# omricarmi/FastHEVC

Hardware: AMD Instinct MI355X
Metric: CTU depth decisions/sec at 1080p all-intra + BD-rate delta vs full-RDO HM (higher is better)
Workload: dtype int8 operands / int32 accumulate on v_mfma_i32_32x32x32_i8 (conv2, conv3: 93 % of the MACs); conv1 bf16 operands / f32 accumulate (fixed-point valued); every result exact

## Files before the change

### fasthevc_amd/csrc/fhevc_api.hip

```cpp
#include "../../include/fasthevc.h"
#include "fhevc_internal.h"

#include <algorithm>
#include <cmath>
#include <cstdio>
#include <cstdlib>
#include <cstring>
#include <functional>
#include <new>
#include <string>
#include <thread>
#include <vector>

namespace {

struct TimedLaunch { hipEvent_t start, stop; int which; };

}

struct fhevc_ctx {
  fhevc_cfg cfg{};
  int device = 0, num_cus = 256;
  hipStream_t stream = nullptr;
  int ctus_x = 0, ctus_y = 0, num_ctus = 0;
  int dev_stride = 0;
  bool have_weights = false;
  uint4* d_frag = nullptr; float* d_bias = nullptr; uint8_t* d_whead = nullptr; int32_t* d_bhead = nullptr;
  uint4* d_frag_i8 = nullptr; int32_t* d_bias_i8 = nullptr;
  bool family = false;
  bool fam_layers = false;
  bool fam_d2 = false;
  FhevcLayersWeights lw = {};
  std::vector<void*> lw_bufs;
  hipEvent_t lw_done = nullptr; hipStream_t lw_last_stream = nullptr; bool lw_in_flight = false;
  int fam_c[3] = { 0, 0, 0 };
  uint4* f_frag1 = nullptr; float* f_bias1 = nullptr; uint4* f_frag2 = nullptr; uint4* f_frag3 = nullptr; int32_t* f_bias_i8 = nullptr;
  uint8_t* f_whead = nullptr; uint8_t* f_headm = nullptr; int32_t* f_bhead = nullptr;
  int shift[3] = { 0, 0, 0 };
  int requant_mode[3] = { 0, 0, 0 };
  bool cnn_i8 = true;
  float scale[3] = { 1, 1, 1 };
  int16_t* d_luma = nullptr; uint8_t* d_depth = nullptr; int32_t* d_had = nullptr; FhevcNodeCost* d_nodes = nullptr;
  int16_t* d_satd = nullptr; uint32_t* d_satd_out = nullptr;
  hipEvent_t ev[4] = { nullptr, nullptr, nullptr, nullptr };
  bool fuse_hadamard = true;
  bool motion_sad = false;
  bool had_valu = true;
  FhevcKnobs knobs;
  bool timing = false;
  std::vector<TimedLaunch> pending;
  std::vector<std::pair<hipEvent_t, hipEvent_t>> pool;
  double sum_ms[5] = { 0, 0, 0, 0, 0 };
  uint64_t launches[5] = { 0, 0, 0, 0, 0 };
  double* d_act = nullptr;
  int16_t* d_pair = nullptr;
  FhevcMotionNode* d_motion = nullptr;
  FhevcNodeCost* d_cand_all = nullptr; uint8_t* d_cand = nullptr;
  uint32_t* d_mvtab = nullptr;
  int mvtab_qp = -1, mvtab_range = -1;
  hipEvent_t mvtab_used = nullptr;
  std::vector<uint32_t> mvtab_host;
  struct Slot {
    hipStream_t st = nullptr;
    uint8_t* d_in = nullptr; uint8_t* d_depth = nullptr; int32_t* d_had = nullptr;
    uint8_t* h_in = nullptr; uint8_t* h_depth = nullptr; int32_t* h_had = nullptr;
    size_t in_cap = 0, frames_cap = 0, h_in_cap = 0;
    int frames = 0; uint8_t* out_depth = nullptr; int32_t* out_had = nullptr; bool staged_out = false;
  } slot[2];
  uint8_t* d_depth_max = nullptr;
  fhevc_stats stats{};
  std::string err;
  std::vector<fhevc_ctx*> peers;
  int fail_peer_for_test = -1;
};

namespace {

int fail(fhevc_ctx* c, int code, const char* what, hipError_t e = hipSuccess)
{
  if (c) {
    c->err = what;
// ... 105 lines not shown
          const int col = 4 * h + (j >> 1), row = 2 * st - 1 + (j & 1);
          uint16_t bits = 0;
          if (c != 0 && row >= 0 && row <= 7) bits = ((__builtin_popcount(u & row) + __builtin_popcount(v & col)) & 1) ? 0xBF80 : 0x3F80;
          frag[((size_t)FHEVC_FRAG_HAD + (mt * 5 + st) * 64 + lane) * 8 + j] = bits;
        }
      }
  std::vector<int8_t> frag8((size_t)FHEVC_FRAGI8_TOTAL * 16, 0);
  for (int lane = 0; lane < 64; ++lane) {
    const int r = lane & 31, h = lane >> 5;
    for (int j = 0; j < 16; ++j) {
      auto w2 = [&](int ky, int kx) { return b.w2[(r * 16 + j) * 9 + ky * 3 + kx]; };
      int8_t* f2 = &frag8[((size_t)FHEVC_FRAGI8_CONV2 + lane) * 16 + j];
      for (int kx = 0; kx < 3; ++kx) f2[(size_t)kx * 1024] = w2(h, kx);
      f2[3 * 1024] = w2(2, 2 * h);
      f2[4 * 1024] = h == 0 ? w2(2, 1) : 0;
      f2[5 * 1024] = h == 1 ? w2(2, 1) : 0;
      for (int t = 0; t < 2; ++t)
        for (int tap = 0; tap < 9; ++tap)
          frag8[((size_t)FHEVC_FRAGI8_CONV3 + (t * 9 + tap) * 64 + lane) * 16 + j] = b.w3[((32 * t + r) * 32 + 16 * h + j) * 9 + tap];
    }
  }
  std::vector<int32_t> bias8(112, 0);
  long long bound[3] = { 0, 0, 0 };
  for (int oc = 0; oc < 32; ++oc) {
    int sw = 0, sa = 0;
    for (int i = 0; i < 16 * 9; ++i) { sw += b.w2[oc * 144 + i]; sa += std::abs((int)b.w2[oc * 144 + i]); }
    bias8[16 + oc] = rd32(b.b2, oc) + 128 * sw;
    bound[1] = std::max(bound[1], (long long)std::abs(bias8[16 + oc]) + 128LL * sa);
  }
  for (int oc = 0; oc < 64; ++oc) {
    int sw = 0, sa = 0;
    for (int i = 0; i < 32 * 9; ++i) { sw += b.w3[oc * 288 + i]; sa += std::abs((int)b.w3[oc * 288 + i]); }
    bias8[48 + oc] = rd32(b.b3, oc) + 128 * sw;
    bound[2] = std::max(bound[2], (long long)std::abs(bias8[48 + oc]) + 128LL * sa);
  }
  for (int l = 1; l < 3; ++l) {
    const int sh = rd32(b.shift, l);
    new_mode[l] = c->knobs.requant_general ? 0 : (sh == 8 && bound[l] < (1LL << 23)) ? 2 : (sh <= 7 ? 1 : 0);
  }
  std::vector<float> bias(112);
  for (int i = 0; i < 16; ++i) {
    int sw = 0;
    for (int t = 0; t < 9; ++t) sw += b.w1[i * 9 + t];
    if (std::abs(rd32(b.b1, i)) > 4194304) return fail(c, FHEVC_E_WEIGHTS, "|bias| > 2^22");
    bias[i] = (float)(rd32(b.b1, i) - 128 * sw);
  }
  for (int i = 0; i < 32; ++i) bias[16 + i] = (float)rd32(b.b2, i);
  for (int i = 0; i < 64; ++i) bias[48 + i] = (float)rd32(b.b3, i);
  for (int i = 16; i < 112; ++i) if (std::fabs(bias[i]) > 4194304.0f) return fail(c, FHEVC_E_WEIGHTS, "|bias| > 2^22");
  std::vector<uint8_t> whead(4 * 4096 + 2 * 1024);
  for (int i = 0; i < 8192; ++i) whead[i] = (uint8_t)b.wh64[i];
  for (int i = 0; i < 8192; ++i) whead[8192 + i] = (uint8_t)b.wh32[i];
  for (int i = 0; i < 2048; ++i) whead[16384 + i] = (uint8_t)b.wh16[i];
  int32_t bhead[6 + 3 * 52] = { rd32(b.bh64, 0), rd32(b.bh64, 1), rd32(b.bh32, 0), rd32(b.bh32, 1), rd32(b.bh16, 0), rd32(b.bh16, 1) };
  for (int cls = 0; cls < 2; ++cls) {
    int s64 = 0, s32 = 0, s16 = 0;
    for (int i = 0; i < 4096; ++i) { s64 += b.wh64[cls * 4096 + i]; s32 += b.wh32[cls * 4096 + i]; }
    for (int i = 0; i < 1024; ++i) s16 += b.wh16[cls * 1024 + i];
    bhead[0 + cls] += 128 * 4 * s64;
    bhead[2 + cls] += 128 * s32;
    bhead[4 + cls] += 128 * s16;
  }
  for (int i = 0; i < 3 * 52; ++i) bhead[6 + i] = rd32(b.qp_bias, i);

  if (c->have_weights && !c->family) c->have_weights = false;
  if (!c->d_frag) {
    HIP_TRY(c, hipMalloc(&c->d_frag, frag.size() * 2));
    HIP_TRY(c, hipMalloc(&c->d_bias, bias.size() * 4));
    HIP_TRY(c, hipMalloc(&c->d_whead, whead.size()));
    HIP_TRY(c, hipMalloc(&c->d_bhead, sizeof bhead));
    HIP_TRY(c, hipMalloc(&c->d_frag_i8, frag8.size()));
    HIP_TRY(c, hipMalloc(&c->d_bias_i8, bias8.size() * 4));
  }
  HIP_TRY(c, hipMemcpy(c->d_frag_i8, frag8.data(), frag8.size(), hipMemcpyHostToDevice));
  HIP_TRY(c, hipMemcpy(c->d_bias_i8, bias8.data(), bias8.size() * 4, hipMemcpyHostToDevice));
  HIP_TRY(c, hipMemcpy(c->d_frag, frag.data(), frag.size() * 2, hipMemcpyHostToDevice));
  HIP_TRY(c, hipMemcpy(c->d_bias, bias.data(), bias.size() * 4, hipMemcpyHostToDevice));
  HIP_TRY(c, hipMemcpy(c->d_whead, whead.data(), whead.size(), hipMemcpyHostToDevice));
  HIP_TRY(c, hipMemcpy(c->d_bhead, bhead, sizeof bhead, hipMemcpyHostToDevice));
  for (int l = 0; l < 3; ++l) { c->shift[l] = new_shift[l]; c->scale[l] = std::ldexp(1.0f, -new_shift[l]); c->requant_mode[l] = new_mode[l]; }
  c->family = false; c->fam_layers = false;
  c->have_weights = true;
  return FHEVC_OK;
}

int build_layers_image(fhevc_ctx* c, const uint8_t* blob, size_t bytes, int C1, int C2, int C3, int depth)
{
  const int C[3] = { C1, C2, C3 };
  for (int b = 0; b < 3; ++b) if (C[b] < 1 || C[b] > 128) return fail(c, FHEVC_E_WEIGHTS, "family widths must be 1..128");
  if (depth < 1 || depth > 3 || (C3 & 3)) return fail(c, FHEVC_E_WEIGHTS, "family members: 1..3 convolutions per block, last width a multiple of 4");
  size_t need = 24 + 36, ci = 1;
  for (int b = 0; b < 3; ++b) for (int j = 0; j < depth; ++j) { need += (size_t)C[b] * ci * 9 + 4 * (size_t)C[b]; ci = (size_t)C[b]; }
  need += (size_t)(2 * 64 + 2 * 64 + 2 * 16) * C3 + 24 + 3 * 52 * 4;
  if (bytes != need) return fail(c, FHEVC_E_WEIGHTS, "FHW3 blob has the wrong size");
  size_t off = 24;
  auto take = [&](size_t n) { const uint8_t* q = blob + off; off += n; return q; };
  auto i32at = [](const uint8_t* p, int i) { int32_t v; std::memcpy(&v, p + 4 * (size_t)i, 4); return v; };
  int32_t shift33[9];
  std::memcpy(shift33, take(36), 36);
  {
    size_t o = off, cin_v = 1;
    for (int b = 0; b < 3; ++b)
      for (int j = 0; j < depth; ++j) {
        const size_t nw = (size_t)C[b] * cin_v * 9;
        for (size_t i = 0; i < nw; ++i) if (static_cast<int8_t>(blob[o + i]) == -128) return fail(c, FHEVC_E_WEIGHTS, "weight -128 not allowed");
        o += nw + 4 * (size_t)C[b];
        cin_v = (size_t)C[b];
        if (shift33[b * 3 + j] < 0 || shift33[b * 3 + j] > 14) return fail(c, FHEVC_E_WEIGHTS, "shift out of range (0..14)");
      }
    const size_t head_bytes[3] = { (size_t)2 * 64 * C3, (size_t)2 * 64 * C3, (size_t)2 * 16 * C3 };
    for (int hd = 0; hd < 3; ++hd) {
      for (size_t i = 0; i < head_bytes[hd]; ++i) if (blob[o + i] == 0x80) return fail(c, FHEVC_E_WEIGHTS, "weight -128 not allowed");
      o += head_bytes[hd] + 8;
    }
  }
  for (void* q : c->lw_bufs) (void)hipFree(q);
  c->lw_bufs.clear();
  if (c->family && c->fam_layers) c->have_weights = false;
  FhevcLayersWeights lw = {};
  lw.chunk = std::min(c->num_ctus * std::max(1, c->cfg.max_frames), 8192);
  if (lw.chunk < 64) lw.chunk = 64;
  auto dev = [&](size_t n, int fill) -> void* { void* q = nullptr; if (hipMalloc(&q, n) != hipSuccess) return nullptr; c->lw_bufs.push_back(q); (void)hipMemset(q, fill, n); return q; };
  auto pad32 = [](int v) { return 32 * ((v + 31) / 32); };
  const bool d2 = depth == 2 && pad32(C1) == 32 && pad32(C2) == 64 && pad32(C3) == 96 && c->knobs.fused_d2 && !c->knobs.family_layers;
  if (!d2 && !(lw.in0 = static_cast<int8_t*>(dev((size_t)lw.chunk * 66 * 66, 0)))) return fail(c, FHEVC_E_HIP, "layer buffers");
  int H = 64, cin = 1, li = 0;
// ... 179 lines not shown
        const int8_t* src;
        if (n < 2) src = wh16 + ((size_t)n * 16 + j) * C3 + 64 * kc;
        else {
          const int sub = (n - 2) >> 1, cls = n & 1, py = j >> 2, px = j & 3;
          src = wh32 + ((size_t)cls * 64 + ((sub >> 1) * 4 + py) * 8 + (sub & 1) * 4 + px) * C3 + 64 * kc;
        }
        std::memcpy(headm.data() + (((size_t)j * KC + kc) * 16 + n) * 64, src, 64);
      }
  int32_t bhead[6 + 3 * 52] = { i32at(bh64p, 0), i32at(bh64p, 1), i32at(bh32p, 0), i32at(bh32p, 1), i32at(bh16p, 0), i32at(bh16p, 1) };
  for (int cls = 0; cls < 2; ++cls) {
    int s64 = 0, s32 = 0, s16 = 0;
    for (int i = 0; i < 64 * C3; ++i) { s64 += wh64[(size_t)cls * 64 * C3 + i]; s32 += wh32[(size_t)cls * 64 * C3 + i]; }
    for (int i = 0; i < 16 * C3; ++i) s16 += wh16[(size_t)cls * 16 * C3 + i];
    bhead[0 + cls] += 128 * 4 * s64;
    bhead[2 + cls] += 128 * s32;
    bhead[4 + cls] += 128 * s16;
  }
  for (int i = 0; i < 3 * 52; ++i) bhead[6 + i] = i32at(qpb, i);
  if (c->family && !c->fam_layers) c->have_weights = false;
  (void)hipFree(c->f_frag1); (void)hipFree(c->f_bias1); (void)hipFree(c->f_frag2); (void)hipFree(c->f_frag3); (void)hipFree(c->f_bias_i8); (void)hipFree(c->f_whead); (void)hipFree(c->f_headm); (void)hipFree(c->f_bhead);
  c->f_frag1 = nullptr; c->f_headm = nullptr; c->f_bias1 = nullptr; c->f_frag2 = nullptr; c->f_frag3 = nullptr; c->f_bias_i8 = nullptr; c->f_whead = nullptr; c->f_bhead = nullptr;
  HIP_TRY(c, hipMalloc(&c->f_frag1, frag1.size() * 2)); HIP_TRY(c, hipMalloc(&c->f_bias1, bias1.size() * 4));
  HIP_TRY(c, hipMalloc(&c->f_frag2, frag2.size())); HIP_TRY(c, hipMalloc(&c->f_frag3, frag3.size()));
  HIP_TRY(c, hipMalloc(&c->f_bias_i8, bias8.size() * 4)); HIP_TRY(c, hipMalloc(&c->f_whead, whead.size())); HIP_TRY(c, hipMalloc(&c->f_headm, headm.size())); HIP_TRY(c, hipMalloc(&c->f_bhead, sizeof bhead));
  HIP_TRY(c, hipMemcpy(c->f_frag1, frag1.data(), frag1.size() * 2, hipMemcpyHostToDevice));
  HIP_TRY(c, hipMemcpy(c->f_bias1, bias1.data(), bias1.size() * 4, hipMemcpyHostToDevice));
  HIP_TRY(c, hipMemcpy(c->f_frag2, frag2.data(), frag2.size(), hipMemcpyHostToDevice));
  HIP_TRY(c, hipMemcpy(c->f_frag3, frag3.data(), frag3.size(), hipMemcpyHostToDevice));
  HIP_TRY(c, hipMemcpy(c->f_bias_i8, bias8.data(), bias8.size() * 4, hipMemcpyHostToDevice));
  HIP_TRY(c, hipMemcpy(c->f_whead, whead.data(), whead.size(), hipMemcpyHostToDevice));
  HIP_TRY(c, hipMemcpy(c->f_headm, headm.data(), headm.size(), hipMemcpyHostToDevice));
  HIP_TRY(c, hipMemcpy(c->f_bhead, bhead, sizeof bhead, hipMemcpyHostToDevice));
  c->fam_c[0] = C1; c->fam_c[1] = C2; c->fam_c[2] = C3;
  c->shift[0] = sh[0]; c->shift[1] = sh[1]; c->shift[2] = sh[2];
  c->family = true; c->fam_layers = false;
  c->have_weights = true;
  return FHEVC_OK;
}

FhevcFamilyWeights family_weights(const fhevc_ctx* c)
{
  FhevcFamilyWeights w;
  w.c[0] = c->fam_c[0]; w.c[1] = c->fam_c[1]; w.c[2] = c->fam_c[2];
  w.frag1 = c->f_frag1; w.bias1 = c->f_bias1; w.frag2 = c->f_frag2; w.frag3 = c->f_frag3; w.bias_i8 = c->f_bias_i8; w.whead = c->f_whead; w.headm = c->f_headm; w.bhead = c->f_bhead;
  w.shift[0] = c->shift[0]; w.shift[1] = c->shift[1]; w.shift[2] = c->shift[2];
  return w;
}

FhevcCnnWeights cnn_weights(const fhevc_ctx* c)
{
  FhevcCnnWeights w;
  w.frag = c->d_frag; w.bias = c->d_bias; w.whead = c->d_whead; w.bhead = c->d_bhead;
  w.scale[0] = c->scale[0]; w.scale[1] = c->scale[1]; w.scale[2] = c->scale[2];
  w.frag_i8 = c->d_frag_i8; w.bias_i8 = c->d_bias_i8;
  w.shift[0] = c->shift[0]; w.shift[1] = c->shift[1]; w.shift[2] = c->shift[2];
  w.requant_mode[0] = 0; w.requant_mode[1] = c->requant_mode[1]; w.requant_mode[2] = c->requant_mode[2];
  w.i8 = c->cnn_i8 ? 1 : 0;
  w.had_valu = c->had_valu ? 1 : 0;
  return w;
}

void time_begin(fhevc_ctx* c, hipStream_t s, int which)
{
  if (!c->timing) return;
  TimedLaunch t;
  if (!c->pool.empty()) { t.start = c->pool.back().first; t.stop = c->pool.back().second; c->pool.pop_back(); }
  else { (void)hipEventCreate(&t.start); (void)hipEventCreate(&t.stop); }
  t.which = which;
  (void)hipEventRecord(t.start, s);
  c->pending.push_back(t);
}
void time_end(fhevc_ctx* c, hipStream_t s)
{
  if (!c->timing) return;
  (void)hipEventRecord(c->pending.back().stop, s);
}
void time_resolve(fhevc_ctx* c)
{
  for (auto& t : c->pending) {
    float ms = 0;
    if (hipEventSynchronize(t.stop) == hipSuccess && hipEventElapsedTime(&ms, t.start, t.stop) == hipSuccess) {
      c->sum_ms[t.which] += ms;
      c->launches[t.which] += 1;
      if (t.which == 0) c->stats.last_cnn_ms = ms;
      if (t.which == 1) c->stats.last_hadamard_ms = ms;
      if (t.which == 2) c->stats.last_first_pass_ms = ms;
    }
    c->pool.emplace_back(t.start, t.stop);
  }
  c->pending.clear();
}

FhevcFrames frames_of(const fhevc_ctx* c, const void* d_luma, int sample_bytes, int stride, long long frame_stride,
                      int num_frames, int row_begin, int row_end, int qp = 32)
{
  FhevcFrames f;
  f.luma = d_luma; f.sample_bytes = sample_bytes; f.stride = stride; f.frame_stride = frame_stride;
  f.width = c->cfg.width; f.height = c->cfg.height; f.bit_depth = c->cfg.bit_depth;
  f.ctus_x = c->ctus_x; f.ctus_y = c->ctus_y; f.num_frames = num_frames; f.row_begin = row_begin; f.row_end = row_end;
  f.qp = qp < 0 ? 0 : (qp > 51 ? 51 : qp);
  return f;
}

}

extern "C" {

// ... 39 lines not shown
  c->ctus_y = (cfg->height + 63) / 64;
  c->num_ctus = c->ctus_x * c->ctus_y;
  c->dev_stride = c->ctus_x * 64;
  if (hipStreamCreateWithFlags(&c->stream, hipStreamDefault) != hipSuccess) { delete c; return FHEVC_E_NO_DEVICE; }
  if (fhevc_cnn_prepare_device() != hipSuccess) { (void)hipStreamDestroy(c->stream); delete c; return FHEVC_E_NO_DEVICE; }
  bool ok = true;
  ok &= hipMalloc(&c->d_luma, (size_t)c->dev_stride * c->ctus_y * 64 * sizeof(int16_t)) == hipSuccess;
  ok &= hipMalloc(&c->d_depth, (size_t)c->num_ctus * 256) == hipSuccess;
  ok &= hipMalloc(&c->d_had, (size_t)c->num_ctus * 4) == hipSuccess;
  ok &= hipMalloc(&c->d_nodes, (size_t)c->num_ctus * FHEVC_NODES_PER_CTU * sizeof(FhevcNodeCost)) == hipSuccess;
  ok &= hipMalloc(&c->d_satd, 2 * 64 * 64 * sizeof(int16_t)) == hipSuccess;
  ok &= hipMalloc(&c->d_satd_out, 4) == hipSuccess;
  for (auto& e : c->ev) ok &= hipEventCreate(&e) == hipSuccess;
  if (!ok) { fhevc_destroy(c); return FHEVC_E_NOMEM; }
  if (hipMemset(c->d_luma, 0, (size_t)c->dev_stride * c->ctus_y * 64 * sizeof(int16_t)) != hipSuccess) { fhevc_destroy(c); return FHEVC_E_HIP; }
  if (cfg->weights_path) {
    FILE* fp = std::fopen(cfg->weights_path, "rb");
    if (!fp) { fhevc_destroy(c); return FHEVC_E_WEIGHTS; }
    std::vector<uint8_t> buf((size_t)4 << 20);
    const size_t n = std::fread(buf.data(), 1, buf.size(), fp);
    std::fclose(fp);
    const int rc = fhevc_set_weights(c, buf.data(), n);
    if (rc != FHEVC_OK) { fhevc_destroy(c); return rc; }
  }
  c->stats.devices = 1;
  for (int d = 1; d < cfg->num_devices; ++d) {
    fhevc_cfg sub = *cfg;
    int id = cfg->device_ids[d];
    sub.num_devices = 1;
    sub.device_ids = &id;
    fhevc_ctx* peer = nullptr;
    if (fhevc_create(&peer, &sub) == FHEVC_OK) { c->peers.push_back(peer); c->stats.devices++; }
    else c->stats.devices_failed++;
  }
  if (const char* ft = std::getenv("FHEVC_TEST_FAIL_DEVICE")) c->fail_peer_for_test = std::atoi(ft);
  (void)hipSetDevice(c->device);
  *out = c;
  return FHEVC_OK;
}

void fhevc_destroy(fhevc_ctx* c)
{
  if (!c) return;
  for (fhevc_ctx* peer : c->peers) fhevc_destroy(peer);
  c->peers.clear();
  (void)hipSetDevice(c->device);
  if (c->stream) (void)hipStreamSynchronize(c->stream);
  time_resolve(c);
  for (auto& p : c->pool) { (void)hipEventDestroy(p.first); (void)hipEventDestroy(p.second); }
  for (auto& e : c->ev) if (e) (void)hipEventDestroy(e);
  if (c->lw_done) (void)hipEventDestroy(c->lw_done);
  if (c->mvtab_used) (void)hipEventDestroy(c->mvtab_used);
  (void)hipFree(c->d_frag); (void)hipFree(c->d_bias); (void)hipFree(c->d_whead); (void)hipFree(c->d_bhead);
  (void)hipFree(c->d_frag_i8); (void)hipFree(c->d_bias_i8);
  (void)hipFree(c->f_frag1); (void)hipFree(c->f_bias1); (void)hipFree(c->f_frag2); (void)hipFree(c->f_frag3); (void)hipFree(c->f_bias_i8); (void)hipFree(c->f_whead); (void)hipFree(c->f_headm); (void)hipFree(c->f_bhead);
  (void)hipFree(c->d_luma); (void)hipFree(c->d_depth); (void)hipFree(c->d_had); (void)hipFree(c->d_nodes); (void)hipFree(c->d_satd); (void)hipFree(c->d_satd_out); (void)hipFree(c->d_act); (void)hipFree(c->d_depth_max); (void)hipFree(c->d_pair); (void)hipFree(c->d_motion); (void)hipFree(c->d_mvtab); (void)hipFree(c->d_cand_all); (void)hipFree(c->d_cand);
  for (void* q : c->lw_bufs) (void)hipFree(q);
  for (auto& sl : c->slot) {
    if (sl.st) { (void)hipStreamSynchronize(sl.st); (void)hipStreamDestroy(sl.st); }
    (void)hipFree(sl.d_in); (void)hipFree(sl.d_depth); (void)hipFree(sl.d_had);
    if (sl.h_in) (void)hipHostFree(sl.h_in);
    if (sl.h_depth) (void)hipHostFree(sl.h_depth);
    if (sl.h_had) (void)hipHostFree(sl.h_had);
  }
  if (c->stream) (void)hipStreamDestroy(c->stream);
  delete c;
}

int fhevc_set_weights(fhevc_ctx* c, const void* blob, size_t bytes)
{
  if (!c || !blob) return FHEVC_E_INVALID;
  auto push_to_peers = [&]() {
    for (fhevc_ctx* peer : c->peers) {
      const int rc = fhevc_set_weights(peer, blob, bytes);
      if (rc != FHEVC_OK) {
        c->have_weights = false;
        for (fhevc_ctx* p2 : c->peers) p2->have_weights = false;
        return fail(c, rc, "weights rejected by a peer device");
      }
    }
    (void)hipSetDevice(c->device);
    return (int)FHEVC_OK;
  };
  (void)hipSetDevice(c->device);
  if (bytes >= 4 && std::memcmp(blob, "FHW3", 4) == 0) {
    const int rc = build_family_image(c, static_cast<const uint8_t*>(blob), bytes);
    return rc != FHEVC_OK ? rc : push_to_peers();
  }
  BlobView v;
  std::vector<uint8_t> copy;
  if (!parse_blob(static_cast<const uint8_t*>(blob), bytes, v, copy)) return fail(c, FHEVC_E_WEIGHTS, "not an FHW1 blob");
  const struct { const int8_t* p; size_t n; } i8s[6] = { { v.w1, 144 }, { v.w2, 4608 }, { v.w3, 18432 }, { v.wh64, 8192 }, { v.wh32, 8192 }, { v.wh16, 2048 } };
  for (const auto& a : i8s)
    for (size_t i = 0; i < a.n; ++i) if (a.p[i] == -128) return fail(c, FHEVC_E_WEIGHTS, "weight -128 not allowed");
  const int rc = build_weight_image(c, v);
  return rc != FHEVC_OK ? rc : push_to_peers();
}

int fhevc_enable_kernel_timing(fhevc_ctx* c, int on)
{
  if (!c) return FHEVC_E_INVALID;
  if (!on) time_resolve(c);
  c->timing = on != 0;
  return FHEVC_OK;
}

int fhevc_kernel_timing(fhevc_ctx* c, int which, int reset, double* avg_ms, uint64_t* launches)
// ... 884 lines not shown
```

### fasthevc_amd/csrc/fhevc_internal.h

```cpp
#pragma once
#include <hip/hip_runtime.h>
#include <stdint.h>

#define FHEVC_CTU 64

#define FHEVC_FRAG_CONV1 0
#define FHEVC_FRAG_CONV2 128
#define FHEVC_FRAG_CONV3 (128 + 9 * 64)
#define FHEVC_FRAG_HAD (128 + 9 * 64 + 2 * 18 * 64)
#define FHEVC_FRAG_TOTAL (FHEVC_FRAG_HAD + 2 * 5 * 64)
#ifndef FHEVC_F16_CONV3_32
#define FHEVC_F16_CONV3_32 0
#endif
#define FHEVC_STAMP_SLOTS 11
#define FHEVC_FRAGI8_CONV2 0
#define FHEVC_FRAGI8_CONV3 (6 * 64)
#define FHEVC_FRAGI8_TOTAL (6 * 64 + 2 * 9 * 64)

struct FhevcKnobs {
  int wg_per_cu = 0;
  int debug_wg_per_cu = 0;
  bool requant_general = false;
  bool family_layers = false;
  bool trio = false;
  bool d2_requant_general = false;
  bool fused_d2 = true;
  bool layers_no_fuse = false;
  bool layers_no_dbuf = false;
  size_t layers_lds_limit = 80 * 1024;
  int layers_grid = 2048;
};
FhevcKnobs fhevc_read_knobs();

struct FhevcFrames {
  const void* luma;
  int sample_bytes;
  int stride;
  long long frame_stride;
  int width, height, bit_depth;
  int ctus_x, ctus_y;
  int num_frames;
  int row_begin, row_end;
  int qp;
};

struct FhevcCnnWeights {
  const uint4* frag;
  const float* bias;
  const uint8_t* whead;
  const int32_t* bhead;
  float scale[3];
  const uint4* frag_i8;
  const int32_t* bias_i8;
  int shift[3];
  int requant_mode[3];
  int i8;
  int had_valu;
};

struct FhevcFamilyWeights {
  int c[3];
  const uint4* frag1;
  const float* bias1;
  const uint4* frag2;
  const uint4* frag3;
  const int32_t* bias_i8;
  const uint8_t* whead;
  const uint8_t* headm;
  const int32_t* bhead;
  int shift[3];
};
hipError_t fhevc_launch_cnn_family(const FhevcFrames& fr, const FhevcFamilyWeights& w, uint8_t* d_depth, int32_t* d_logits, uint32_t* d_flags,
                                   uint8_t* d_depth_max, int margin_split, int margin_stop, int num_cus, hipStream_t stream);
bool fhevc_cnn_family_supported(int c1, int c2, int c3);

struct FhevcLayer {
  const uint4* frag;
  const int32_t* bias;
  int8_t* out;
  int shift, kc, cout_pad, H, pool;
  int rq;
  int in_pad, out_pad, swz;
};
void fhevc_layer_lds_image(int kc, int pool, int H, int* pad, int* mask);
struct FhevcLayersWeights {
  int num_layers, chunk, c3, c3_pad;
  int d2_short;
  FhevcLayer l[9];
  int8_t* in0;
  const uint8_t* whead;
  const int32_t* bhead;
};

hipError_t fhevc_launch_cnn_layers(const FhevcFrames& fr, const FhevcLayersWeights& w, uint8_t* d_depth, int32_t* d_logits, uint32_t* d_flags,
                                   uint8_t* d_depth_max, int margin_split, int margin_stop, int num_cus, const FhevcKnobs& knobs, hipStream_t stream);

bool fhevc_cnn_d2_supported(const FhevcLayersWeights& w);
hipError_t fhevc_launch_cnn_d2(const FhevcFrames& fr, const FhevcLayersWeights& w, uint8_t* d_depth, int32_t* d_logits, uint32_t* d_flags,
                               uint8_t* d_depth_max, int margin_split, int margin_stop, int num_cus, hipStream_t stream);

hipError_t fhevc_cnn_prepare_device();
bool fhevc_cnn_can_fuse_hadamard(const FhevcFrames& fr);
hipError_t fhevc_launch_cnn(const FhevcFrames& fr, const FhevcCnnWeights& w, uint8_t* d_depth, int32_t* d_had, int32_t* d_logits,
                            uint32_t* d_flags, uint8_t* d_depth_max, int margin_split, int margin_stop, int num_cus, const FhevcKnobs& knobs, hipStream_t stream);
hipError_t fhevc_launch_expand_flags(const FhevcFrames& fr, const uint32_t* d_flags, uint8_t* d_depth, hipStream_t stream);

// ... 36 lines not shown
```

### fasthevc_amd/csrc/k_cnn.hip

```cpp
#include "fhevc_internal.h"
#include <algorithm>
#include <cstdlib>
#include <cstring>

typedef __attribute__((ext_vector_type(8))) short bf16x8;
typedef __attribute__((ext_vector_type(8))) _Float16 f16x8;
typedef __attribute__((ext_vector_type(16))) float f32x16;
typedef __attribute__((ext_vector_type(2))) unsigned short u16x2;

namespace {

constexpr int A1_ROW = 36 * 16;
constexpr int A1_EVEN = 19 * 16;
constexpr int R1_OFF = 0;
constexpr int A3_OFF = R1_OFF;
constexpr int A2_PITCH = 18;
constexpr int A2_PLANE = 18 * 18 * 16 + 192;
constexpr int IN_PITCH = 68;
#ifndef FHEVC_I8_PRIO
#define FHEVC_I8_PRIO 0x0222
#endif
#ifndef FHEVC_F16_PRIO
#define FHEVC_F16_PRIO 0x0123
#endif
// ... 552 lines not shown
  const u16x2 sh = { (unsigned short)shift, (unsigned short)shift };
  t = __builtin_bit_cast(s16x2, (u16x2)((__builtin_bit_cast(u16x2, t) + __builtin_bit_cast(u16x2, rnd2)) >> sh));
  t = __builtin_elementwise_min(t, top);
  return __builtin_bit_cast(unsigned, t);
}

template <bool HALO = true>
__device__ __forceinline__ void stage_ctu(unsigned char* lds, int r2_off, const Prefetched& pre, const FhevcFrames& F, CtuPos c,
                                          int tid, int ld_row, int ld_seg, int shift_in, unsigned in_cells)
{
  unsigned short* inh = reinterpret_cast<unsigned short*>(lds + r2_off);
  const int hy = ld_row + 1;
  unsigned short* dst = inh + 2 * ((hy >> 1) * IN_PITCH + ld_seg * 16 + 1) + (hy & 1);
  if (pre.fast) {
    if (F.sample_bytes == 2) {
      const unsigned wds[8] = { pre.a.x, pre.a.y, pre.a.z, pre.a.w, pre.b.x, pre.b.y, pre.b.z, pre.b.w };
      const unsigned rnd2 = shift_in > 0 ? (0x00010001u << (shift_in - 1)) : 0u;
#pragma unroll
      for (int j = 0; j < 8; ++j) {
        const unsigned t = sample8_pair(wds[j], shift_in, rnd2);
        dst[4 * j] = (unsigned short)(__float_as_uint((float)(t & 0xFF)) >> 16);
        dst[4 * j + 2] = (unsigned short)(__float_as_uint((float)((t >> 16) & 0xFF)) >> 16);
      }
    } else {
      const unsigned wds[4] = { pre.a.x, pre.a.y, pre.a.z, pre.a.w };
#pragma unroll
      for (int j = 0; j < 16; ++j) {
        const unsigned v = (wds[j >> 2] >> (8 * (j & 3))) & 0xFF;
        dst[2 * j] = (unsigned short)(__float_as_uint((float)v) >> 16);
      }
    }
  } else {
    const int f = c.f, cy = F.row_begin + c.ry, cx = c.cx;
    const int py = cy * 64 + ld_row, px0 = cx * 64 + ld_seg * 16;
    const long long base = (long long)f * F.frame_stride + (long long)py * F.stride + px0;
    const bool row_ok = py < F.height;
#pragma unroll 4
    for (int j = 0; j < 16; ++j) {
      int v = 128;
      if (row_ok && px0 + j < F.width) {
        if (F.sample_bytes == 2) v = load_sample8(reinterpret_cast<const int16_t*>(F.luma) + base + j, shift_in);
        else v = (int)reinterpret_cast<const uint8_t*>(F.luma)[base + j];
      }
      dst[2 * j] = (unsigned short)(__float_as_uint((float)v) >> 16);
    }
  }
  if (HALO) {
    asm volatile("" : "+v"(in_cells));
    *reinterpret_cast<unsigned short*>(lds + (in_cells & 0xFFFF)) = 0x4300;
    if (tid < 260 - 256) *reinterpret_cast<unsigned short*>(lds + (in_cells >> 16)) = 0x4300;
  }
}
template <bool I8>
__device__ __forceinline__ int a1_halo_off(int e)
{
  const int pl = e / 132, k0 = e - pl * 132;
  int y, x;
  if (k0 < 34) { y = 0; x = k0; }
  else if (k0 < 68) { y = 33; x = k0 - 34; }
  else { const int k = k0 - 68; y = 1 + (k >> 1); x = (k & 1) ? 33 : 0; }
  return R1_OFF + pl * Lds<I8>::A1_PLANE + y * A1_ROW + ((x & 1) ? 0 : A1_EVEN) + (x >> 1) * 16;
}
template <bool I8>
__device__ __forceinline__ int a2_halo_off(int e)
{
  const int pl = e / 68, k0 = e - pl * 68;
  int y, x;
  if (k0 < 18) { y = 0; x = k0; }
  else if (k0 < 36) { y = 17; x = k0 - 18; }
  else { const int k = k0 - 36; y = 1 + (k >> 1); x = (k & 1) ? 17 : 0; }
  return Lds<I8>::R2_OFF + pl * A2_PLANE + (y * A2_PITCH + x) * 16;
}
template <bool I8>
__device__ __forceinline__ int in_halo_off(int e)
{
  int y, x;
  if (e < 66) { y = 0; x = e; }
  else if (e < 132) { y = 65; x = e - 66; }
  else { const int k = e - 132; y = 1 + (k >> 1); x = (k & 1) ? 65 : 0; }
  return Lds<I8>::R2_OFF + 2 * (2 * ((y >> 1) * IN_PITCH + x) + (y & 1));
}
struct HaloCells { unsigned a1, a2, in; };
template <bool I8>
__device__ __forceinline__ HaloCells halo_cells(int tid)
{
  constexpr int N1 = 132 * Lds<I8>::A1_PLANES, N2 = 68 * Lds<I8>::A2_PLANES;
  HaloCells hc;
  hc.a1 = (unsigned)a1_halo_off<I8>(min(tid, N1 - 1)) | ((unsigned)a1_halo_off<I8>(min(tid + 256, N1 - 1)) << 16);
  hc.a2 = (unsigned)a2_halo_off<I8>(min(tid, N2 - 1)) | ((unsigned)a2_halo_off<I8>(min(tid + 256, N2 - 1)) << 16);
  hc.in = (unsigned)in_halo_off<I8>(tid) | ((unsigned)in_halo_off<I8>(min(tid + 256, 259)) << 16);
  return hc;
}
template <bool I8>
__device__ __forceinline__ void zero_a1_halo(unsigned char* lds, int tid, unsigned cells)
{
  asm volatile("" : "+v"(cells));
  constexpr unsigned Z = Lds<I8>::HALO_FILL;
  *reinterpret_cast<uint4*>(lds + (cells & 0xFFFF)) = make_uint4(Z, Z, Z, Z);
  if (tid < 132 * Lds<I8>::A1_PLANES - 256) *reinterpret_cast<uint4*>(lds + (cells >> 16)) = make_uint4(Z, Z, Z, Z);
}

__device__ __forceinline__ unsigned long long stamp()
{
  unsigned long long t;
  __builtin_amdgcn_sched_barrier(0);
  asm volatile("s_memtime %0\n\ts_waitcnt lgkmcnt(0)" : "=s"(t)::"memory");
  __builtin_amdgcn_sched_barrier(0);
  return t;
}

#define FHEVC_PHASE_IDS                                   \
  int tid = (int)threadIdx.x;                             \
  asm volatile("" : "+v"(tid));                           \
  if (TRIO) tid &= 255;                                   \
  const int lane = tid & 63, wave = tid >> 6;             \
  const int r = lane & 31, h = lane >> 5;                 \
  (void)r; (void)h; (void)wave;

template <bool STAMPS, int HAD, int ARITH, int TRIO = 0>
__global__ __launch_bounds__(TRIO ? 768 : 256, TRIO ? 1 : (ARITH ? FHEVC_I8_WG_PER_CU : 2)) void fhevc_cnn_depth_kernel(FhevcFrames F, FhevcCnnWeights W,
                                                                  uint8_t* __restrict__ d_depth, int32_t* __restrict__ d_had,
                                                                  int32_t* __restrict__ d_logits,
                                                                  uint32_t* __restrict__ d_flags,
                                                                  unsigned long long* __restrict__ d_stamps,
                                                                  uint8_t* __restrict__ d_depth_max, int margin_split, int margin_stop)
{
  extern __shared__ __attribute__((aligned(16))) unsigned char lds_all[];
  const int group = TRIO ? __builtin_amdgcn_readfirstlane((int)(threadIdx.x >> 8)) : 0;
  unsigned char* const lds = lds_all + (TRIO ? group * Lds<ARITH != 0>::LDS_BYTES : 0);
  const int vgrid = TRIO ? 3 * (int)gridDim.x : (int)gridDim.x;
  const int vbidx = TRIO ? group * (int)gridDim.x + (int)blockIdx.x : (int)blockIdx.x;
  __builtin_amdgcn_s_setreg((1 << 11) | 1, 2);
  const int tid = TRIO ? (int)(threadIdx.x & 255) : (int)threadIdx.x;
  const int lane = tid & 63, wave = tid >> 6;
  constexpr bool I8 = ARITH != 0, FASTRQ = ARITH == 2;
  int prio_slot = 0;
  if (I8) {
    const unsigned la = __builtin_amdgcn_s_getreg((31 << 11) | 6);
    const unsigned base = la & 0xFFFu, sz = (la >> 12) & 0x1FFu;
    prio_slot = base >= 2 * sz && sz ? 2 : (base >= sz && sz ? 1 : 0);
    if (TRIO) prio_slot = group;
  }
  (void)prio_slot;
  constexpr bool MFMA_HEADS = I8;
  (void)FASTRQ;
  using L = Lds<I8>;
  const HaloCells hc = halo_cells<I8>(tid);
  const int hb64a = W.bhead[0], hb64b = W.bhead[1] + W.bhead[6 + 0 * 52 + F.qp];
  const int hb32a = W.bhead[2], hb32b = W.bhead[3] + W.bhead[6 + 1 * 52 + F.qp];
  const int hb16a = W.bhead[4], hb16b = W.bhead[5] + W.bhead[6 + 2 * 52 + F.qp];
  const uint4* frag1p = W.frag + FHEVC_FRAG_CONV1 + lane;
  bf16x8 wA1a = __builtin_bit_cast(bf16x8, frag1p[0]);
  bf16x8 wA1b = __builtin_bit_cast(bf16x8, frag1p[64]);
  bf16x8 wA2[9];
  bf16x8 wA3[18];
  const int tile3 = wave & 1;
  if (I8) {
#pragma unroll
    for (int s = 0; s < 6; ++s) wA2[s] = __builtin_bit_cast(bf16x8, W.frag_i8[FHEVC_FRAGI8_CONV2 + s * 64 + lane]);
#pragma unroll
    for (int s = 0; s < 9; ++s) wA3[s] = __builtin_bit_cast(bf16x8, W.frag_i8[FHEVC_FRAGI8_CONV3 + (tile3 * 9 + s) * 64 + lane]);
  } else {
#pragma unroll
    for (int s = 0; s < 9; ++s) wA2[s] = __builtin_bit_cast(bf16x8, W.frag[FHEVC_FRAG_CONV2 + s * 64 + lane]);
#pragma unroll
    for (int s = 0; s < 18; ++s) wA3[s] = __builtin_bit_cast(bf16x8, W.frag[FHEVC_FRAG_CONV3 + (tile3 * 18 + s) * 64 + lane]);
  }
  const int shift2 = W.shift[1], shift3 = W.shift[2];
  (void)shift2; (void)shift3;

  float* biasL = reinterpret_cast<float*>(lds + L::BIAS_OFF);
  int* logitL = reinterpret_cast<int*>(lds + L::LOGIT_OFF);
  if (tid < 112) {
    if (I8 && tid >= 16) {
      reinterpret_cast<int*>(biasL)[tid] = W.bias_i8[tid];
    } else {
      float b = W.bias[tid];
      b *= (tid < 16 ? W.scale[0] : (tid < 48 ? W.scale[1] : W.scale[2]));
      biasL[tid] = b;
    }
  }
  for (int i = tid; i < (MFMA_HEADS ? 8192 : 18432) / 16; i += 256) {
    const int row = i >> 2, c = i & 3;
    const int sw = (i < 2 * 4096 * 2 / 16) ? ((row >> 3) & 3) : ((row >> 2) & 3);
    *reinterpret_cast<uint4*>(lds + L::HEADW_OFF + row * 64 + ((c ^ sw) << 4)) = reinterpret_cast<const uint4*>(W.whead)[i];
  }
  if (MFMA_HEADS) {
    for (int i = tid; i < HEADM_BYTES / 16; i += 256) {
      const int j = i / 40, rem = i - j * 40, n = rem >> 2, kg = rem & 3;
      int src;
      if (n < 2) src = 16384 + (n * 16 + j) * 64;
      else {
        const int sub = (n - 2) >> 1, cls = n & 1, py = j >> 2, px = j & 3;
        src = 8192 + (cls * 64 + ((sub >> 1) * 4 + py) * 8 + (sub & 1) * 4 + px) * 64;
      }
      *reinterpret_cast<uint4*>(lds + L::HEADW_OFF + HEADM_OFF + i * 16) = *reinterpret_cast<const uint4*>(W.whead + src + kg * 16);
    }
  }

  if (MFMA_HEADS && tid < 64) {
    const int n = tid & 15, rg = tid >> 4, subn = (n - 2) >> 1;
    const bool is16 = n < 2, is32 = n >= 2 && n < 10 && ((rg & 1) == (subn >> 1));
    unsigned a[4];
    for (int i = 0; i < 4; ++i) {
      const bool act = is16 || (is32 && ((i & 1) == (subn & 1)));
      const int idx = is16 ? 2 * (5 + 4 * rg + i) + n : 2 * (1 + (rg >> 1) * 2 + (i >> 1)) + (n & 1);
      a[i] = act ? (unsigned)(L::LOGIT_OFF + 4 * idx) : (unsigned)(L::HEADX_OFF + 512 + 4 * tid);
    }
    *reinterpret_cast<uint2*>(lds + L::HEADX_OFF + tid * 8) = make_uint2(a[0] | (a[1] << 16), a[2] | (a[3] << 16));
  }
  const int band_rows = F.row_end - F.row_begin;
  const int per_frame = band_rows * F.ctus_x;
  const int total = per_frame * F.num_frames;
  const int shift_in = F.bit_depth - 8;

  unsigned long long tsum[8] = { 0, 0, 0, 0, 0, 0, 0, 0 }, tprev = 0;
#define FHEVC_STAMP(k)                                     \
  if (STAMPS) {                                            \
    const unsigned long long tn = stamp();                 \
    tsum[k] += tn - tprev;                                 \
    tprev = tn;                                            \
  }
  unsigned long long tclk0 = 0, treal0 = 0;
  if (STAMPS) {
    tprev = stamp();
    tclk0 = tprev;
    asm volatile("s_memrealtime %0\n\ts_waitcnt lgkmcnt(0)" : "=s"(treal0)::"memory");
  }

  const int ld_row = tid >> 2, ld_seg = tid & 3;
  const int vblock = (vgrid & 7) ? vbidx : ((vbidx & 7) * (vgrid >> 3) + (vbidx >> 3));
  CtuPos pos, step;
  {
    const int vb = min(vblock, total - 1), g = vgrid;
    pos.f = vb / per_frame; pos.ry = (vb - pos.f * per_frame) / F.ctus_x; pos.cx = (vb - pos.f * per_frame) - pos.ry * F.ctus_x;
    step.f = g / per_frame; step.ry = (g - step.f * per_frame) / F.ctus_x; step.cx = (g - step.f * per_frame) - step.ry * F.ctus_x;
  }
  Prefetched pre = prefetch_ctu<HAD == 1>(F, vblock < total, pos, ld_row, ld_seg);
  uint2 head_addr;
  {
    const int q = wave, blk = lane >> 4;
    const int y = (q >> 1) * 8 + (blk >> 1) * 4 + ((lane >> 2) & 3), x = (q & 1) * 8 + (blk & 1) * 4 + (lane & 3);
    const unsigned psw = (x >> 2) & 3, sw16 = y & 3, sw32 = y & 3, sw64 = (y >> 1) & 3;
    const unsigned a_0 = (unsigned)(y * 16 + x) * 64 + (psw << 4);
    const unsigned w16_0 = (unsigned)((y & 3) * 4 + (x & 3)) * 64 + (sw16 << 4);
    const unsigned w32_0 = (unsigned)((y & 7) * 8 + (x & 7)) * 64 + (sw32 << 4);
    const unsigned w64_0 = (unsigned)((y >> 1) * 8 + (x >> 1)) * 64 + (sw64 << 4);
    head_addr = make_uint2(a_0 | (w16_0 << 16), w32_0 | (w64_0 << 16));
  }
  unsigned headm_addr = 0;
  if (MFMA_HEADS) {
    const int m = lane & 15, kg = lane >> 4, by = m >> 2, bx = m & 3;
    const unsigned am = (unsigned)((4 * by + wave) * 16 + 4 * bx) * 64 + ((unsigned)(kg ^ bx) << 4);
    const unsigned bm = (unsigned)(HEADM_OFF + 4 * wave * HEADM_STEP + min(m, 9) * 64 + 16 * kg);
    headm_addr = am | (bm << 16);
  }
  (void)headm_addr;
  int had_set = 0;
  if (vblock < total) {
    stage_ctu(lds, L::R2_OFF, pre, F, pos, tid, ld_row, ld_seg, shift_in, hc.in);
    zero_a1_halo<I8>(lds, tid, hc.a1);
    if (HAD == 1) {
      const int hs = F.sample_bytes == 2 ? wave_src_hadamard<2>(pre, lane) : wave_src_hadamard<1>(pre, lane);
      if (lane == 0) logitL[56 + wave] = hs;
    }
  }
  __syncthreads();
  FHEVC_STAMP(0)
  float4 early_b0, early_b1;
  bf16x8 early_bq;
#define FHEVC_CONV1_EARLY_READS                                                                          \
  {                                                                                                      \
    FHEVC_PHASE_IDS                                                                                      \
    early_b0 = *reinterpret_cast<const float4*>(biasL + 8 * h);                                          \
    early_b1 = *reinterpret_cast<const float4*>(biasL + 8 * h + 4);                                      \
    const unsigned char* p = lds + L::R2_OFF + (2 * r + 2 * h) * 4 + wave * (IN_PITCH * 4);              \
    const uint2 lo = *reinterpret_cast<const uint2*>(p);                                                 \
    const uint2 hi = *reinterpret_cast<const uint2*>(p + IN_PITCH * 4);                                  \
    early_bq = __builtin_bit_cast(bf16x8, make_uint4(lo.x, lo.y, hi.x, hi.y));                           \
  }
  FHEVC_CONV1_EARLY_READS
  bf16x8 wH[5];
#define FHEVC_HAD_FRAG_LOADS                                                                                                              \
  if (HAD == 2) {                                                                                                                         \
    unsigned hoff = (unsigned)(threadIdx.x & 63) * 16u + (unsigned)((threadIdx.x >> 6) & 1) * (5u * 64u * 16u);   \
    asm volatile("" : "+v"(hoff));                                                                                                        \
    const unsigned char* hf = reinterpret_cast<const unsigned char*>(W.frag + FHEVC_FRAG_HAD) + hoff;                                     \
    _Pragma("unroll") for (int st = 0; st < 5; ++st) wH[st] = __builtin_bit_cast(bf16x8, *reinterpret_cast<const uint4*>(hf + st * 64 * 16)); \
  }
  FHEVC_HAD_FRAG_LOADS

  if (TRIO) {
    for (int i = 0; i < group; ++i) __syncthreads();
  }
  const int trio_iters = TRIO ? (total + vgrid - 1) / vgrid : 0;
  for (int work = vblock, it = 0; TRIO ? it < trio_iters : work < total; work += vgrid, ++it) {
    if (TRIO && work >= total) {
      __syncthreads(); __syncthreads(); __syncthreads(); __syncthreads();
      continue;
    }
    const int f = pos.f, cy = F.row_begin + pos.ry, cx = pos.cx;
    const CtuPos next = advance(pos, step, band_rows, F.ctus_x);


    {
      FHEVC_PHASE_IDS
      FHEVC_PRIO_ON(0)
      const unsigned char* inb = lds + L::R2_OFF + (2 * r + 2 * h) * 4;
      f32x16 bias1;
      {
        const float4 b0 = early_b0, b1 = early_b1;
        bias1[0] = b0.x; bias1[1] = b0.y; bias1[2] = b0.z; bias1[3] = b0.w;
        bias1[4] = b1.x; bias1[5] = b1.y; bias1[6] = b1.z; bias1[7] = b1.w;
#pragma unroll
        for (int i = 0; i < 8; ++i) bias1[8 + i] = bias1[i];
      }
      auto frag1 = [](const unsigned char* p) {
        const uint2 lo = *reinterpret_cast<const uint2*>(p);
        const uint2 hi = *reinterpret_cast<const uint2*>(p + IN_PITCH * 4);
// ... 714 lines not shown
```

Baseline: 85.81 million.

## Pre-swizzle head weights on host and DMA them into LDS with global_load_lds

The MFMA-heads path now receives a head-weight image whose swizzle is computed once on the host. It is copied into LDS with direct global-to-LDS loads, replacing the per-thread load/swizzle/store loops. Halo offsets and head-index tables become constexpr device tables instead of being computed per thread. The CTU prefetch is moved earlier so it overlaps with weight staging. The cost is an extra device buffer and a full vmcnt wait before the first barrier, which may serialize the prefetch.

```diff
diff --git a/fasthevc_amd/csrc/fhevc_api.hip b/fasthevc_amd/csrc/fhevc_api.hip
--- a/fasthevc_amd/csrc/fhevc_api.hip
+++ b/fasthevc_amd/csrc/fhevc_api.hip
@@ -27,6 +27,7 @@
   bool have_weights = false;
   uint4* d_frag = nullptr; float* d_bias = nullptr; uint8_t* d_whead = nullptr; int32_t* d_bhead = nullptr;
   uint4* d_frag_i8 = nullptr; int32_t* d_bias_i8 = nullptr;
+  uint4* d_headimg = nullptr;
   bool family = false;
   bool fam_layers = false;
   bool fam_d2 = false;
@@ -238,6 +239,21 @@
   for (int i = 0; i < 8192; ++i) whead[i] = (uint8_t)b.wh64[i];
   for (int i = 0; i < 8192; ++i) whead[8192 + i] = (uint8_t)b.wh32[i];
   for (int i = 0; i < 2048; ++i) whead[16384 + i] = (uint8_t)b.wh16[i];
+  std::vector<uint8_t> headimg(FHEVC_HEADIMG_BYTES);
+  for (int i = 0; i < 8192 / 16; ++i) {
+    const int row = i >> 2, ch = i & 3, sw = (row >> 3) & 3;
+    std::memcpy(headimg.data() + row * 64 + ((ch ^ sw) << 4), whead.data() + 16 * i, 16);
+  }
+  for (int j = 0; j < 16; ++j)
+    for (int n = 0; n < 10; ++n) {
+      int src;
+      if (n < 2) src = 16384 + (n * 16 + j) * 64;
+      else {
+        const int sub = (n - 2) >> 1, cls = n & 1, py = j >> 2, px = j & 3;
+        src = 8192 + (cls * 64 + ((sub >> 1) * 4 + py) * 8 + (sub & 1) * 4 + px) * 64;
+      }
+      std::memcpy(headimg.data() + 8192 + (j * 10 + n) * 64, whead.data() + src, 64);
+    }
   int32_t bhead[6 + 3 * 52] = { rd32(b.bh64, 0), rd32(b.bh64, 1), rd32(b.bh32, 0), rd32(b.bh32, 1), rd32(b.bh16, 0), rd32(b.bh16, 1) };
   for (int cls = 0; cls < 2; ++cls) {
     int s64 = 0, s32 = 0, s16 = 0;
@@ -258,6 +274,8 @@
     HIP_TRY(c, hipMalloc(&c->d_frag_i8, frag8.size()));
     HIP_TRY(c, hipMalloc(&c->d_bias_i8, bias8.size() * 4));
   }
+  if (!c->d_headimg) HIP_TRY(c, hipMalloc(&c->d_headimg, headimg.size()));
+  HIP_TRY(c, hipMemcpy(c->d_headimg, headimg.data(), headimg.size(), hipMemcpyHostToDevice));
   HIP_TRY(c, hipMemcpy(c->d_frag_i8, frag8.data(), frag8.size(), hipMemcpyHostToDevice));
   HIP_TRY(c, hipMemcpy(c->d_bias_i8, bias8.data(), bias8.size() * 4, hipMemcpyHostToDevice));
   HIP_TRY(c, hipMemcpy(c->d_frag, frag.data(), frag.size() * 2, hipMemcpyHostToDevice));
@@ -543,7 +561,7 @@
   FhevcCnnWeights w;
   w.frag = c->d_frag; w.bias = c->d_bias; w.whead = c->d_whead; w.bhead = c->d_bhead;
   w.scale[0] = c->scale[0]; w.scale[1] = c->scale[1]; w.scale[2] = c->scale[2];
-  w.frag_i8 = c->d_frag_i8; w.bias_i8 = c->d_bias_i8;
+  w.frag_i8 = c->d_frag_i8; w.bias_i8 = c->d_bias_i8; w.headimg = c->d_headimg;
   w.shift[0] = c->shift[0]; w.shift[1] = c->shift[1]; w.shift[2] = c->shift[2];
   w.requant_mode[0] = 0; w.requant_mode[1] = c->requant_mode[1]; w.requant_mode[2] = c->requant_mode[2];
   w.i8 = c->cnn_i8 ? 1 : 0;
@@ -689,7 +707,7 @@
   if (c->lw_done) (void)hipEventDestroy(c->lw_done);
   if (c->mvtab_used) (void)hipEventDestroy(c->mvtab_used);
   (void)hipFree(c->d_frag); (void)hipFree(c->d_bias); (void)hipFree(c->d_whead); (void)hipFree(c->d_bhead);
-  (void)hipFree(c->d_frag_i8); (void)hipFree(c->d_bias_i8);
+  (void)hipFree(c->d_frag_i8); (void)hipFree(c->d_bias_i8); (void)hipFree(c->d_headimg);
   (void)hipFree(c->f_frag1); (void)hipFree(c->f_bias1); (void)hipFree(c->f_frag2); (void)hipFree(c->f_frag3); (void)hipFree(c->f_bias_i8); (void)hipFree(c->f_whead); (void)hipFree(c->f_headm); (void)hipFree(c->f_bhead);
   (void)hipFree(c->d_luma); (void)hipFree(c->d_depth); (void)hipFree(c->d_had); (void)hipFree(c->d_nodes); (void)hipFree(c->d_satd); (void)hipFree(c->d_satd_out); (void)hipFree(c->d_act); (void)hipFree(c->d_depth_max); (void)hipFree(c->d_pair); (void)hipFree(c->d_motion); (void)hipFree(c->d_mvtab); (void)hipFree(c->d_cand_all); (void)hipFree(c->d_cand);
   for (void* q : c->lw_bufs) (void)hipFree(q);
diff --git a/fasthevc_amd/csrc/fhevc_internal.h b/fasthevc_amd/csrc/fhevc_internal.h
--- a/fasthevc_amd/csrc/fhevc_internal.h
+++ b/fasthevc_amd/csrc/fhevc_internal.h
@@ -16,6 +16,7 @@
 #define FHEVC_FRAGI8_CONV2 0
 #define FHEVC_FRAGI8_CONV3 (6 * 64)
 #define FHEVC_FRAGI8_TOTAL (6 * 64 + 2 * 9 * 64)
+#define FHEVC_HEADIMG_BYTES 18432
 
 struct FhevcKnobs {
   int wg_per_cu = 0;
@@ -52,6 +53,7 @@
   float scale[3];
   const uint4* frag_i8;
   const int32_t* bias_i8;
+  const uint4* headimg;
   int shift[3];
   int requant_mode[3];
   int i8;
diff --git a/fasthevc_amd/csrc/k_cnn.hip b/fasthevc_amd/csrc/k_cnn.hip
--- a/fasthevc_amd/csrc/k_cnn.hip
+++ b/fasthevc_amd/csrc/k_cnn.hip
@@ -628,7 +628,7 @@
   }
 }
 template <bool I8>
-__device__ __forceinline__ int a1_halo_off(int e)
+constexpr int a1_halo_off(int e)
 {
   const int pl = e / 132, k0 = e - pl * 132;
   int y, x;
@@ -638,7 +638,7 @@
   return R1_OFF + pl * Lds<I8>::A1_PLANE + y * A1_ROW + ((x & 1) ? 0 : A1_EVEN) + (x >> 1) * 16;
 }
 template <bool I8>
-__device__ __forceinline__ int a2_halo_off(int e)
+constexpr int a2_halo_off(int e)
 {
   const int pl = e / 68, k0 = e - pl * 68;
   int y, x;
@@ -648,7 +648,7 @@
   return Lds<I8>::R2_OFF + pl * A2_PLANE + (y * A2_PITCH + x) * 16;
 }
 template <bool I8>
-__device__ __forceinline__ int in_halo_off(int e)
+constexpr int in_halo_off(int e)
 {
   int y, x;
   if (e < 66) { y = 0; x = e; }
@@ -657,15 +657,41 @@
   return Lds<I8>::R2_OFF + 2 * (2 * ((y >> 1) * IN_PITCH + x) + (y & 1));
 }
 struct HaloCells { unsigned a1, a2, in; };
+constexpr int cmin(int a, int b) { return a < b ? a : b; }
 template <bool I8>
-__device__ __forceinline__ HaloCells halo_cells(int tid)
-{
-  constexpr int N1 = 132 * Lds<I8>::A1_PLANES, N2 = 68 * Lds<I8>::A2_PLANES;
-  HaloCells hc;
-  hc.a1 = (unsigned)a1_halo_off<I8>(min(tid, N1 - 1)) | ((unsigned)a1_halo_off<I8>(min(tid + 256, N1 - 1)) << 16);
-  hc.a2 = (unsigned)a2_halo_off<I8>(min(tid, N2 - 1)) | ((unsigned)a2_halo_off<I8>(min(tid + 256, N2 - 1)) << 16);
-  hc.in = (unsigned)in_halo_off<I8>(tid) | ((unsigned)in_halo_off<I8>(min(tid + 256, 259)) << 16);
-  return hc;
+struct PrologueTables {
+  unsigned halo[3][256];
+  unsigned headx[128];
+  constexpr PrologueTables() : halo{}, headx{}
+  {
+    using L = Lds<I8>;
+    constexpr int N1 = 132 * L::A1_PLANES, N2 = 68 * L::A2_PLANES;
+    for (int t = 0; t < 256; ++t) {
+      halo[0][t] = (unsigned)a1_halo_off<I8>(cmin(t, N1 - 1)) | ((unsigned)a1_halo_off<I8>(cmin(t + 256, N1 - 1)) << 16);
+      halo[1][t] = (unsigned)a2_halo_off<I8>(cmin(t, N2 - 1)) | ((unsigned)a2_halo_off<I8>(cmin(t + 256, N2 - 1)) << 16);
+      halo[2][t] = (unsigned)in_halo_off<I8>(t) | ((unsigned)in_halo_off<I8>(cmin(t + 256, 259)) << 16);
+    }
+    for (int t = 0; t < 64; ++t) {
+      const int n = t & 15, rg = t >> 4, subn = (n - 2) >> 1;
+      const bool is16 = n < 2, is32 = n >= 2 && n < 10 && ((rg & 1) == (subn >> 1));
+      unsigned a[4] = { 0, 0, 0, 0 };
+      for (int i = 0; i < 4; ++i) {
+        const bool act = is16 || (is32 && ((i & 1) == (subn & 1)));
+        const int idx = is16 ? 2 * (5 + 4 * rg + i) + n : 2 * (1 + (rg >> 1) * 2 + (i >> 1)) + (n & 1);
+        a[i] = act ? (unsigned)(L::LOGIT_OFF + 4 * idx) : (unsigned)(L::HEADX_OFF + 512 + 4 * t);
+      }
+      headx[2 * t] = a[0] | (a[1] << 16);
+      headx[2 * t + 1] = a[2] | (a[3] << 16);
+    }
+  }
+};
+__device__ constexpr PrologueTables<false> k_prologue_f16{};
+__device__ constexpr PrologueTables<true> k_prologue_i8{};
+template <bool I8>
+__device__ __forceinline__ const PrologueTables<I8>& prologue_tables()
+{
+  if constexpr (I8) return k_prologue_i8;
+  else return k_prologue_f16;
 }
 template <bool I8>
 __device__ __forceinline__ void zero_a1_halo(unsigned char* lds, int tid, unsigned cells)
@@ -721,7 +747,8 @@
   constexpr bool MFMA_HEADS = I8;
   (void)FASTRQ;
   using L = Lds<I8>;
-  const HaloCells hc = halo_cells<I8>(tid);
+  const PrologueTables<I8>& tab = prologue_tables<I8>();
+  const HaloCells hc = { tab.halo[0][tid], tab.halo[1][tid], tab.halo[2][tid] };
   const int hb64a = W.bhead[0], hb64b = W.bhead[1] + W.bhead[6 + 0 * 52 + F.qp];
   const int hb32a = W.bhead[2], hb32b = W.bhead[3] + W.bhead[6 + 1 * 52 + F.qp];
   const int hb16a = W.bhead[4], hb16b = W.bhead[5] + W.bhead[6 + 2 * 52 + F.qp];
@@ -745,6 +772,20 @@
   const int shift2 = W.shift[1], shift3 = W.shift[2];
   (void)shift2; (void)shift3;
 
+  const int band_rows = F.row_end - F.row_begin;
+  const int per_frame = band_rows * F.ctus_x;
+  const int total = per_frame * F.num_frames;
+  const int shift_in = F.bit_depth - 8;
+
+  const int ld_row = tid >> 2, ld_seg = tid & 3;
+  const int vblock = (vgrid & 7) ? vbidx : ((vbidx & 7) * (vgrid >> 3) + (vbidx >> 3));
+  CtuPos pos, step;
+  {
+    const int vb = min(vblock, total - 1), g = vgrid;
+    pos.f = vb / per_frame; pos.ry = (vb - pos.f * per_frame) / F.ctus_x; pos.cx = (vb - pos.f * per_frame) - pos.ry * F.ctus_x;
+    step.f = g / per_frame; step.ry = (g - step.f * per_frame) / F.ctus_x; step.cx = (g - step.f * per_frame) - step.ry * F.ctus_x;
+  }
+  Prefetched pre = prefetch_ctu<HAD == 1>(F, vblock < total, pos, ld_row, ld_seg);
   float* biasL = reinterpret_cast<float*>(lds + L::BIAS_OFF);
   int* logitL = reinterpret_cast<int*>(lds + L::LOGIT_OFF);
   if (tid < 112) {
@@ -756,39 +797,19 @@
       biasL[tid] = b;
     }
   }
-  for (int i = tid; i < (MFMA_HEADS ? 8192 : 18432) / 16; i += 256) {
-    const int row = i >> 2, c = i & 3;
-    const int sw = (i < 2 * 4096 * 2 / 16) ? ((row >> 3) & 3) : ((row >> 2) & 3);
-    *reinterpret_cast<uint4*>(lds + L::HEADW_OFF + row * 64 + ((c ^ sw) << 4)) = reinterpret_cast<const uint4*>(W.whead)[i];
-  }
   if (MFMA_HEADS) {
-    for (int i = tid; i < HEADM_BYTES / 16; i += 256) {
-      const int j = i / 40, rem = i - j * 40, n = rem >> 2, kg = rem & 3;
-      int src;
-      if (n < 2) src = 16384 + (n * 16 + j) * 64;
-      else {
-        const int sub = (n - 2) >> 1, cls = n & 1, py = j >> 2, px = j & 3;
-        src = 8192 + (cls * 64 + ((sub >> 1) * 4 + py) * 8 + (sub & 1) * 4 + px) * 64;
-      }
-      *reinterpret_cast<uint4*>(lds + L::HEADW_OFF + HEADM_OFF + i * 16) = *reinterpret_cast<const uint4*>(W.whead + src + kg * 16);
-    }
-  }
-
-  if (MFMA_HEADS && tid < 64) {
-    const int n = tid & 15, rg = tid >> 4, subn = (n - 2) >> 1;
-    const bool is16 = n < 2, is32 = n >= 2 && n < 10 && ((rg & 1) == (subn >> 1));
-    unsigned a[4];
-    for (int i = 0; i < 4; ++i) {
-      const bool act = is16 || (is32 && ((i & 1) == (subn & 1)));
-      const int idx = is16 ? 2 * (5 + 4 * rg + i) + n : 2 * (1 + (rg >> 1) * 2 + (i >> 1)) + (n & 1);
-      a[i] = act ? (unsigned)(L::LOGIT_OFF + 4 * idx) : (unsigned)(L::HEADX_OFF + 512 + 4 * tid);
-    }
-    *reinterpret_cast<uint2*>(lds + L::HEADX_OFF + tid * 8) = make_uint2(a[0] | (a[1] << 16), a[2] | (a[3] << 16));
-  }
-  const int band_rows = F.row_end - F.row_begin;
-  const int per_frame = band_rows * F.ctus_x;
-  const int total = per_frame * F.num_frames;
-  const int shift_in = F.bit_depth - 8;
+    const int wv = __builtin_amdgcn_readfirstlane(wave);
+    for (int k = wv; k < FHEVC_HEADIMG_BYTES / 1024; k += 4)
+      __builtin_amdgcn_global_load_lds((const void __attribute__((address_space(1)))*)(W.headimg + k * 64 + lane),
+                                       (void __attribute__((address_space(3)))*)(lds + L::HEADW_OFF + k * 1024), 16, 0, 0);
+    if (tid < 64) *reinterpret_cast<uint2*>(lds + L::HEADX_OFF + tid * 8) = make_uint2(tab.headx[2 * tid], tab.headx[2 * tid + 1]);
+  } else {
+    for (int i = tid; i < 18432 / 16; i += 256) {
+      const int row = i >> 2, c = i & 3;
+      const int sw = (i < 2 * 4096 * 2 / 16) ? ((row >> 3) & 3) : ((row >> 2) & 3);
+      *reinterpret_cast<uint4*>(lds + L::HEADW_OFF + row * 64 + ((c ^ sw) << 4)) = reinterpret_cast<const uint4*>(W.whead)[i];
+    }
+  }
 
   unsigned long long tsum[8] = { 0, 0, 0, 0, 0, 0, 0, 0 }, tprev = 0;
 #define FHEVC_STAMP(k)                                     \
@@ -804,15 +825,6 @@
     asm volatile("s_memrealtime %0\n\ts_waitcnt lgkmcnt(0)" : "=s"(treal0)::"memory");
   }
 
-  const int ld_row = tid >> 2, ld_seg = tid & 3;
-  const int vblock = (vgrid & 7) ? vbidx : ((vbidx & 7) * (vgrid >> 3) + (vbidx >> 3));
-  CtuPos pos, step;
-  {
-    const int vb = min(vblock, total - 1), g = vgrid;
-    pos.f = vb / per_frame; pos.ry = (vb - pos.f * per_frame) / F.ctus_x; pos.cx = (vb - pos.f * per_frame) - pos.ry * F.ctus_x;
-    step.f = g / per_frame; step.ry = (g - step.f * per_frame) / F.ctus_x; step.cx = (g - step.f * per_frame) - step.ry * F.ctus_x;
-  }
-  Prefetched pre = prefetch_ctu<HAD == 1>(F, vblock < total, pos, ld_row, ld_seg);
   uint2 head_addr;
   {
     const int q = wave, blk = lane >> 4;
@@ -841,6 +853,7 @@
       if (lane == 0) logitL[56 + wave] = hs;
     }
   }
+  if (MFMA_HEADS) asm volatile("s_waitcnt vmcnt(0)" ::: "memory");
   __syncthreads();
   FHEVC_STAMP(0)
   float4 early_b0, early_b1;
```

Result: no change. 86.13 million, median of 6 (+0.4%).
